# jinli99/iShapEditing

Hardware: AMD Instinct MI355X
Metric: end-to-end drag-edit wall-clock (s) per shape (lower is better)
Workload: dtype f16

## Files before the change

### ishapediting_amd/csrc/igemm.hip

```cpp
#include "common.h"
#include "igemm_epilogue.h"
#include "gn_bwd_terms.h"

template <int BM, int BN, int BK, int WM, int WN, bool CONV3>
__global__ __launch_bounds__(256) void igemm_kernel(IgemmArgs a) {
  constexpr int CPR = BK / 8;
  constexpr int XL = BM * CPR / 256;
  constexpr int WL = BN * CPR / 256;
  constexpr int TMW = BM / WM, TNW = BN / WN;
  constexpr int MT = TMW / 16, NT = TNW / 16;
  static_assert(XL >= 1 && WL >= 1, "tile too small for 256 threads");
  extern __shared__ __attribute__((aligned(16))) char smem_raw[];
  half_t* sX = reinterpret_cast<half_t*>(smem_raw);
  half_t* sW = sX + 2 * BM * BK;

  const int tid = threadIdx.x;
  const int lane = tid & 63;
  const int wave = tid >> 6;
  const int wm = wave / WN, wn = wave % WN;
  const int m0 = blockIdx.x * BM;
  const int n0 = blockIdx.y * BN;
  const int batch = blockIdx.z / a.ksplit;
  const int ks_id = blockIdx.z % a.ksplit;

// ... 220 lines not shown
  hipEvent_t e;
  (void)hipEventCreate(&e);
  return e;
}
extern "C" int ishap_profile_begin(void) {
  for (auto& r : g_prof) { g_prof_pool.push_back(r.a); g_prof_pool.push_back(r.b); if (r.c) g_prof_pool.push_back(r.c); }
  g_prof.clear();
  g_prof_on = true;
  return 0;
}
extern "C" int ishap_profile_end(double* out, int nvar) {
  g_prof_on = false;
  for (int i = 0; i < nvar * 3; ++i) out[i] = 0.0;
  for (auto& r : g_prof) {
    if (hipEventSynchronize(r.b) != hipSuccess) return -1;
    float ms = 0.f;
    if (hipEventElapsedTime(&ms, r.a, r.b) != hipSuccess) return -1;
    if (r.variant < nvar) { out[r.variant * 3] += 1.0; out[r.variant * 3 + 1] += ms; out[r.variant * 3 + 2] += r.flops; }
  }
  return 0;
}

#include <map>
#include <cstring>
#include <array>
#include <string>
extern "C" int ishap_profile_shapes(char* buf, int cap) {
  std::map<std::array<int, 6>, std::array<double, 4>> agg;
  for (auto& r : g_prof) {
    if (hipEventSynchronize(r.c ? r.c : r.b) != hipSuccess) return -1;
    float ms = 0.f, ms2 = 0.f;
    if (hipEventElapsedTime(&ms, r.a, r.b) != hipSuccess) return -1;
    if (r.c && hipEventElapsedTime(&ms2, r.b, r.c) != hipSuccess) return -1;
    auto& v = agg[{r.M, r.N, r.K, r.conv3, r.big ? 128 : 64, r.ksplit}];
    v[0] += 1.0; v[1] += ms; v[2] += ms2; v[3] += r.flops * 1e-9;
  }
  std::string out;
  char line[160];
  for (auto& kv : agg) {
    snprintf(line, sizeof line, "%d,%d,%d,%d,%d,%d,%.0f,%.4f,%.4f,%.3f\n", kv.first[0], kv.first[1], kv.first[2], kv.first[3],
             kv.first[4], kv.first[5], kv.second[0], kv.second[1], kv.second[2], kv.second[3]);
    out += line;
  }
  if ((int)out.size() + 1 > cap) return -2;
  memcpy(buf, out.c_str(), out.size() + 1);
  return (int)agg.size();
}

int igemm2_launch_main(const IgemmArgs& a, bool big, hipStream_t s);
bool igemm2_two_teams(const IgemmArgs& a, bool big);
bool igemm4_applicable(const IgemmArgs& a, bool big);
bool igemm4_two_teams(const IgemmArgs& a, bool big);
bool igemm4_tall_tiles(const IgemmArgs& a, bool big);
int igemm4_launch_main(const IgemmArgs& a, bool big, hipStream_t s);
static bool igemm4_wanted(const IgemmArgs& a, bool big) {
  static const int use4 = [] { const char* e = getenv("ISHAP_IGEMM4"); return e ? atoi(e) : 2; }();
  return use4 && (use4 > 1 || big) && igemm4_applicable(a, big);
}

template <int BM, int BN, int BK, int WM, int WN, bool CONV3>
static int launch_cfg(const IgemmArgs& a, hipStream_t s) {
  int prof_slot = -1;
  auto fire = [&]() -> int {
    if constexpr (BK == 64) {
      if (CONV3 && igemm4_wanted(a, BM == 128)) return igemm4_launch_main(a, BM == 128, s);
      return igemm2_launch_main(a, BM == 128, s);
    } else {
      constexpr size_t smem = 2 * (size_t)(BM + BN) * BK * sizeof(half_t);
      auto kern = igemm_kernel<BM, BN, BK, WM, WN, CONV3>;
      ISHAP_TRY(ishap_set_max_lds((const void*)kern, (int)smem));
      const dim3 grid(a.M / BM, ceil_div(a.N, BN), a.nbatch * a.ksplit);
      if (g_igemm_prof_start) hipExtLaunchKernelGGL(kern, grid, dim3(256), smem, s, g_igemm_prof_start, g_igemm_prof_stop, 0, a);
      else hipLaunchKernelGGL(kern, grid, dim3(256), smem, s, a);
      return 0;
    }
  };
  if (g_prof_on) {
    ProfRec r;
    r.a = prof_event(); r.b = prof_event(); r.c = nullptr;
    r.flops = 2.0 * a.M * a.N * a.K * a.nbatch * a.flops_scale;
    r.variant = BK == 64 ? ((CONV3 ? 0 : 2) + (BM == 128 ? 0 : 1)) : 6;
    if (BK == 64 && igemm2_two_teams(a, BM == 128)) r.variant = 4;
    if (BK == 64 && CONV3 && igemm4_wanted(a, BM == 128))
      r.variant = BM == 128 ? 8 : (a.W == 8 ? 11 : (igemm4_tall_tiles(a, false) ? 12 : (igemm4_two_teams(a, false) ? 10 : 9)));
    r.M = a.M * a.nbatch; r.N = a.N; r.K = a.K; r.conv3 = CONV3; r.big = BM == 128; r.ksplit = a.ksplit;
    g_igemm_prof_start = r.a; g_igemm_prof_stop = r.b;
    const int rc = fire();
    g_igemm_prof_start = nullptr; g_igemm_prof_stop = nullptr;
    if (rc) return rc;
    prof_slot = (int)g_prof.size();
    g_prof.push_back(r);
  } else {
    ISHAP_TRY(fire());
  }
  ISHAP_CHECK_HIP(hipGetLastError());
  if (a.ksplit > 1 && !a.defer_reduce) {
    const unsigned rblocks = (unsigned)((long long)a.nbatch * (a.M / 16) * ((a.N + 63) / 64));
    hipLaunchKernelGGL(igemm_splitk_reduce, dim3(rblocks), dim3(256), 0, s, a);
    ISHAP_CHECK_HIP(hipGetLastError());
    if (prof_slot >= 0) {
      g_prof[prof_slot].c = prof_event();
      (void)hipEventRecord(g_prof[prof_slot].c, s);
    }
  }
  return 0;
}

static bool igemm_use_big(int M, int N, int nbatch) {
  if (M % 128 != 0 || N < 128) return false;
  long long blocks = (long long)(M / 128) * ceil_div(N, 128) * nbatch;
  static const int big_min = [] { const char* e = getenv("ISHAP_BIG_MIN"); return e ? atoi(e) : 192; }();
  return blocks >= big_min;
}
int igemm_pick_ksplit(int M, int N, int K, int nbatch, bool pending) {
  const bool big = igemm_use_big(M, N, nbatch);
  const int bm = big ? 128 : 64, bn = big ? 128 : 64;
  long long blocks = (long long)(M / bm) * ceil_div(N, bn) * nbatch;
  int ks = K / 64;
  constexpr int nosplit = 36;
  constexpr int fill = 224;
  constexpr int minsteps = 6;
  constexpr int p_nosplit = 12, p_minsteps = 3;
  if (ks < (pending ? p_nosplit : nosplit)) return 1;
  int split = 1;
  while (blocks * split < fill && ks / (split * 2) >= (pending ? p_minsteps : minsteps) && split < 32) split *= 2;
  return split;
}

int igemm_reduce_launch(const IgemmArgs& a, hipStream_t s) {
  ISHAP_REQUIRE(a.ksplit > 1 && a.ws && a.M % 16 == 0 && a.N % 4 == 0, "reduce: split-K slices of a finished launch");
  const unsigned rblocks = (unsigned)((long long)a.nbatch * (a.M / 16) * ((a.N + 63) / 64));
  hipLaunchKernelGGL(igemm_splitk_reduce, dim3(rblocks), dim3(256), 0, s, a);
  ISHAP_CHECK_HIP(hipGetLastError());
  return 0;
}

bool igemm_skinny_applicable(const IgemmArgs& a);
// ... 57 lines not shown
```

### ishapediting_amd/csrc/igemm4.hip

```cpp
#include "common.h"
#include "igemm_epilogue.h"
#include <type_traits>

__device__ __attribute__((aligned(128))) half_t g_zero_line4[64];
typedef __attribute__((address_space(3))) void lds_void4;

constexpr int ig4_loads(int a, int b, int wi, int xi) {
  int c = 0;
  for (int u = a; u <= b; ++u) c += wi + ((u % 3 == 0) ? xi : 0);
  return c;
}

#ifndef IG4_PRO
#define IG4_PRO 2
#endif

#ifdef ABL_NOLOAD
#define IG4_DMA(src, dst) asm volatile("" ::"v"(src), "v"((unsigned)(unsigned long long)(lds_void4*)(dst)))
#else
#define IG4_DMA(src, dst) __builtin_amdgcn_global_load_lds((src), (lds_void4*)(dst), 16, 0, 0)
#endif

__device__ __forceinline__ void ig4_wait_vm(int n) {
#define IG4_W(k) case k: asm volatile("s_waitcnt vmcnt(" #k ")" ::: "memory"); break;
  switch (n) {
    IG4_W(0) IG4_W(1) IG4_W(2) IG4_W(3) IG4_W(4) IG4_W(5) IG4_W(6) IG4_W(7) IG4_W(8) IG4_W(9) IG4_W(10) IG4_W(11) IG4_W(12)
    IG4_W(13) IG4_W(14) IG4_W(15) IG4_W(16) IG4_W(17) IG4_W(18) IG4_W(19) IG4_W(20) IG4_W(21) IG4_W(22) IG4_W(23) IG4_W(24)
    IG4_W(25) IG4_W(26) IG4_W(27) IG4_W(28) IG4_W(29) IG4_W(30) IG4_W(31) IG4_W(32) IG4_W(33) IG4_W(34) IG4_W(35) IG4_W(36)
    IG4_W(37) IG4_W(38) IG4_W(39) IG4_W(40)
    default: asm volatile("s_waitcnt vmcnt(0)" ::: "memory"); break;
  }
#undef IG4_W
}

template <int BM, int BN, int WD, int NSTW, int NSTX, int HALVES = 1>
__global__ __launch_bounds__(512 * HALVES) void igemm4_kernel(const void* hX, const void* hWt, int hK, int hCin, int hldx, int hldw, int hH, int hW,
                                                              int hksplit, int hnwg, unsigned hpacked, int hbase, IgemmArgs a) {
  const IgemmHot h{(const half_t*)hX, (const half_t*)hWt, hK, hCin, hldx, hldw, hH, hW, hksplit, hnwg, hpacked};
#if defined(__HIP_DEVICE_COMPILE__)
  constexpr int BK = 64;
  constexpr int XI = BM / 8 / 4;
  constexpr int WI = BN / 8 / 4;
  constexpr int WSLOT = BN * BK;
  constexpr int XSLOT = (BM + 8) * BK;
  constexpr int RING = NSTW * WSLOT + NSTX * XSLOT;
  constexpr int TMW = BM / 2, TNW = BN / 2, MT = TMW / 16, NT = TNW / 16;
  constexpr int DIST = NSTW - 1;
  constexpr int PRO = DIST < IG4_PRO ? DIST : IG4_PRO;
  constexpr int RAMP = DIST - PRO;
  static_assert(RAMP <= 6, "ramp iterations are peeled by hand");
  static_assert(NSTX * 3 >= DIST + 3, "activation ring too shallow for the prefetch distance");
  static_assert(BM % WD == 0, "a tile is whole image rows (fragment addresses are per lane, so a 16-pixel MFMA sub-tile may span rows)");
  static_assert(DIST * (WI + XI) <= 40, "ig4_wait_vm covers up to 40 outstanding loads");
  extern __shared__ __attribute__((aligned(16))) char smem_raw[];

  const int tid = threadIdx.x, lane = tid & 63;
  const int wave_all = __builtin_amdgcn_readfirstlane(tid >> 6);
  const int team = HALVES == 2 ? wave_all >> 3 : 0;
  const int wave8 = wave_all & 7;
  half_t* const sW = reinterpret_cast<half_t*>(smem_raw) + team * RING;
  half_t* const sX = sW + NSTW * WSLOT;
  const bool loader = wave8 >= 4;
  const int wave = wave8 & 3;
  const int wm = wave >> 1, wn = wave & 1;
  IG_STAMP(0, wave_all == 0);
  if (tid < HALVES * NSTX * 8) {
    const int tm = tid / (NSTX * 8), k = tid - tm * (NSTX * 8);
    *reinterpret_cast<f32x4*>(reinterpret_cast<half_t*>(smem_raw) + tm * RING + NSTW * WSLOT + (k >> 3) * XSLOT + BM * BK + (k & 7) * 8) =
        (f32x4){0.f, 0.f, 0.f, 0.f};
  }
  int tile_m, tile_n, tile_z;
  {
    const int nx = h.ny_shift() >= 0 ? (1 << h.nx_shift()) : (int)gridDim.x, ny = h.ny_shift() >= 0 ? (1 << h.ny_shift()) : (int)gridDim.y;
    const int nwg = h.nwg;
    const bool n_outer = (hbase >> 30) & 1;
    const int lin = (hbase & 0x3fffffff) + blockIdx.x + nx * (blockIdx.y + ny * blockIdx.z);
    const int q = nwg >> 3, r = nwg & 7, xcd = lin & 7, pos = lin >> 3;
    const int swz = (xcd < r ? xcd * (q + 1) : r * (q + 1) + (xcd - r) * q) + pos;
    if (n_outer) {
      tile_m = swz & (nx - 1);
      const int rest = swz >> h.nx_shift();
      tile_n = rest / h.ksplit;
      tile_z = rest - tile_n * h.ksplit;
    } else if (h.ny_shift() >= 0) {
      tile_n = swz & (ny - 1);
      tile_m = (swz >> h.ny_shift()) & (nx - 1);
      tile_z = swz >> (h.ny_shift() + h.nx_shift());
    } else {
      tile_n = swz % ny;
      tile_m = (swz / ny) % nx;
      tile_z = swz / (ny * nx);
    }
  }
  const int m0 = tile_m * BM, n0 = tile_n * BN;
  const int ks_id = tile_z;
  const int H = h.H, HW = H * WD;
  const int NC = h.Cin / BK;
  const int NC2 = (int)(h.packed >> 25);
  const int G = 3 * NC;
  const int per = (G + h.ksplit - 1) / h.ksplit, per2 = (NC2 + h.ksplit - 1) / h.ksplit;
  int g0 = min(G, ks_id * per), g1 = min(G, g0 + per);
  int c20 = min(NC2, ks_id * per2), c21 = min(NC2, c20 + per2);
  int nk_loop = (g1 - g0) * 3 + (c21 - c20);
  if (HALVES == 2) {
    const int ga = min(g1 - g0, (nk_loop + 3) / 6);
    const int n0s = ga * 3, n1s = nk_loop - n0s;
    nk_loop = max(n0s, n1s);
    if (team == 0) { g1 = g0 + ga; c21 = c20; }
    else g0 += ga;
  }
  const int ns3 = (g1 - g0) * 3, ns = ns3 + (c21 - c20);
  const int n_img = h.hw_shift() >= 0 ? (m0 >> h.hw_shift()) : m0 / HW;
  const int y0 = (m0 - n_img * HW) / WD;
  __syncthreads();

  f32x4 acc[NT][MT];
#pragma unroll
  for (int i = 0; i < NT; ++i)
#pragma unroll
    for (int j = 0; j < MT; ++j) acc[i][j] = (f32x4){0.f, 0.f, 0.f, 0.f};

  IG_STAMP(1, wave_all == 0);
  if (loader) {
    const int lrow = lane >> 3, pch = lane & 7;
    int hc = g0 / 3, hdy = g0 - hc * 3, hdx = 0;
    const half_t* xp[XI];
    const half_t* zp[XI];
    int yr[XI], xc[XI];
#pragma unroll
    for (int i = 0; i < XI; ++i) {
      const int row = (wave * XI + i) * 8 + lrow;
      yr[i] = y0 + row / WD;
      xc[i] = row % WD;
      const int sc = (pch ^ (row & 7)) * 8;
      zp[i] = (const half_t*)g_zero_line4 + sc;
      xp[i] = h.X + ((long long)n_img * HW + (long long)(yr[i] + hdy - 1) * WD + xc[i]) * h.ldx + hc * BK + sc;
    }
    const long long x_row = (long long)WD * h.ldx;
    const half_t* wp[WI];
#pragma unroll
    for (int i = 0; i < WI; ++i) {
      const int row = (wave * WI + i) * 8 + lrow;
      wp[i] = h.Wt + (long long)(n0 + row) * h.ldw + (pch ^ ((row >> 1) & 7)) * 8 + (long long)(3 * hdy) * h.Cin + hc * BK;
    }
    int hws = 0, hxs = 0;
    int issued = 0, tot = 0;
// ... 258 lines not shown
          if (decltype(SLAB_ENDS)::value && s + 1 >= ns3) read_half(integral_constant<int, 1>{}, 0, sw_off, sx_off, xa, wa);
          else read_half(integral_constant<int, (d + 1) % 3>{}, 0, sw_off, sx_off, xa, wa);
        }
        __builtin_amdgcn_sched_barrier(0);
      }
      mfma_half(xb, wb);
    };
    auto step = [&](auto DX, auto SLAB_ENDS, int s) __attribute__((always_inline)) {
      if constexpr (INTERLEAVE) step_il(DX, SLAB_ENDS, s);
      else step_burst(DX, SLAB_ENDS, s);
    };
    if (nk_loop > 0) __builtin_amdgcn_s_barrier();
    asm volatile("" ::: "memory");
    IG_STAMP(2, wave_all == 0);
    if (ns > 0) {
      if (ns3 > 0) read_half(integral_constant<int, 0>{}, 0, sw_off, sx_off, xa, wa);
      else read_half(integral_constant<int, 1>{}, 0, sw_off, sx_off, xa, wa);
    }
    int s = 0;
    for (; s < ns3; s += 3) {
      step(integral_constant<int, 0>{}, std::false_type{}, s);
      step(integral_constant<int, 1>{}, std::false_type{}, s + 1);
      step(integral_constant<int, 2>{}, std::true_type{}, s + 2);
    }
    for (; s < ns; ++s) step(integral_constant<int, 1>{}, std::true_type{}, s);
    for (; s < nk_loop; ++s)
      if (s + 1 < nk_loop) __builtin_amdgcn_s_barrier();
  }
  IG_STAMP(3, wave_all == 0);
  const bool merge_in_epilogue = HALVES == 2 && igemm_epilogue_is_staged(a, 0);
  if (HALVES == 2 && !merge_in_epilogue) {
    f32x4* red = reinterpret_cast<f32x4*>(reinterpret_cast<half_t*>(smem_raw) + RING);
    __syncthreads();
    if (!loader && team == 1) {
#pragma unroll
      for (int i = 0; i < NT; ++i)
#pragma unroll
        for (int j = 0; j < MT; ++j) red[((i * MT + j) * 4 + wave) * 64 + lane] = acc[i][j];
    }
    __syncthreads();
    if (!loader && team == 0) {
#pragma unroll
      for (int i = 0; i < NT; ++i)
#pragma unroll
        for (int j = 0; j < MT; ++j) acc[i][j] += red[((i * MT + j) * 4 + wave) * 64 + lane];
    }
  }
  IG_STAMP(4, wave_all == 0);
  igemm_epilogue<MT, NT, TMW, TNW, BN, 512 * HALVES>(a, acc, m0, n0, wm, wn, lane, 0, ks_id, reinterpret_cast<float*>(smem_raw),
                                                     !loader && (team == 0 || merge_in_epilogue), merge_in_epilogue ? team : -1);
#endif
}

template <int BM, int BN, int WD, int NSTW, int NSTX, int HALVES = 1>
static int launch4(const IgemmArgs& a, hipStream_t s) {
  constexpr size_t ring = (size_t)HALVES * (NSTW * BN * 64 + NSTX * (BM + 8) * 64) * sizeof(half_t);
  constexpr size_t epi = (size_t)HALVES * BM * (BN + 4) * 4 + (size_t)BM * (BN + 8) * 2 + 16384;
  static_assert((ring > epi ? ring : epi) <= 163840, "LDS");
  const size_t smem = ring > epi ? ring : epi;
  auto kern = igemm4_kernel<BM, BN, WD, NSTW, NSTX, HALVES>;
  ISHAP_TRY(ishap_set_max_lds((const void*)kern, (int)smem));
  const dim3 grid(a.M / BM, ceil_div(a.N, BN), a.ksplit);
  IgemmArgs b = a;
  auto lg2 = [](int v) { int k = 0; while ((1 << k) < v) ++k; return (1 << k) == v ? k : -1; };
  b.w_shift = lg2(a.W);
  b.hw_shift = lg2(a.H * a.W);
  if (b.w_shift < 0 || b.hw_shift < 0) b.w_shift = b.hw_shift = -1;
  b.nx_shift = lg2((int)grid.x);
  b.ny_shift = lg2((int)grid.y);
  if (b.nx_shift < 0 || b.ny_shift < 0) b.nx_shift = b.ny_shift = -1;
  IgemmHot h;
  h.X = b.X; h.Wt = b.Wt; h.K = b.K; h.Cin = b.Cin; h.ldx = b.ldx; h.ldw = b.ldw; h.H = b.H; h.W = b.W; h.ksplit = b.ksplit;
  h.nwg = (int)(grid.x * grid.y * grid.z);
  h.packed = (unsigned)(b.w_shift & 0x3f) | (unsigned)(b.hw_shift & 0x3f) << 6 | (unsigned)(b.nx_shift & 0x3f) << 12 |
             (unsigned)(b.ny_shift & 0x3f) << 18 | (b.ups ? 1u << 24 : 0u) | (unsigned)(b.K2 / 64) << 25;
  int n_outer = 0;
  if (b.nx_shift >= 0) {
    static const int force = [] { const char* e = getenv("ISHAP_IG4_NOUTER"); return e ? atoi(e) : 2; }();
    const int nx = (int)grid.x, ny = (int)grid.y, nz = (int)grid.z;
    const int q = (h.nwg + 7) / 8;
    const double wp = (double)BN * (b.K / (double)nz) * 2.0;
    const double xs = (double)BM * b.Cin * 2.0 / nz + (b.K2 ? (double)BM * b.K2 * 2.0 / nz : 0.0);
    auto cdiv = [](int a, int d) { return (a + d - 1) / d; };
    const int nA = ny < q ? ny : q, mzA = cdiv(q, ny), mA = nx < mzA ? nx : mzA, zA = cdiv(mzA, nx);
    const double costA = (double)nA * zA * wp + (double)mA * zA * xs;
    const int mB = nx < q ? nx : q, znB = cdiv(q, nx), zB = nz < znB ? nz : znB;
    const double costB = (double)znB * wp + (double)mB * zB * xs;
    n_outer = force == 2 ? (costB < 0.8 * costA) : force;
  }
  const int order_bit = n_outer ? (1 << 30) : 0;
  const int tiles = h.nwg;
  const int chunk = a.chunk_tiles;
  const bool chunked = chunk > 0 && chunk % 8 == 0 && tiles > chunk && b.nx_shift >= 0 && !g_igemm_prof_start;
  if (chunked) {
    for (int base = 0; base < tiles; base += chunk) {
      const int n = tiles - base < chunk ? tiles - base : chunk;
      hipLaunchKernelGGL(kern, dim3(n), dim3(512 * HALVES), smem, s,
                         (const void*)h.X, (const void*)h.Wt, h.K, h.Cin, h.ldx, h.ldw, h.H, h.W, h.ksplit, h.nwg, h.packed, base | order_bit, b);
    }
  } else if (g_igemm_prof_start) hipExtLaunchKernelGGL(kern, grid, dim3(512 * HALVES), smem, s, g_igemm_prof_start, g_igemm_prof_stop, 0,
                                                (const void*)h.X, (const void*)h.Wt, h.K, h.Cin, h.ldx, h.ldw, h.H, h.W, h.ksplit, h.nwg, h.packed, order_bit, b);
  else hipLaunchKernelGGL(kern, grid, dim3(512 * HALVES), smem, s,
                          (const void*)h.X, (const void*)h.Wt, h.K, h.Cin, h.ldx, h.ldw, h.H, h.W, h.ksplit, h.nwg, h.packed, order_bit, b);
  ISHAP_CHECK_HIP(hipGetLastError());
  return 0;
}

bool igemm4_applicable(const IgemmArgs& a, bool big) {
  const int BM = big ? 128 : 64;
  if (!a.conv3 || a.nbatch != 1 || a.Cin % 64 != 0 || a.K != 9 * a.Cin + a.K2) return false;
  if (a.K2 && (a.K2 % 64 != 0 || a.K2 / 64 > 127 || !a.X2)) return false;
  const bool w8 = !big && a.W == 8 && a.H == 8 && a.ksplit > 1;
  if (a.K2 && !big && !w8) return false;
  if (big ? (a.W != 128 && a.W != 64 && a.W != 32 && a.W != 16) : (a.W != 16 && a.W != 32 && a.W != 64 && !w8)) return false;
  if (BM % a.W != 0 || (a.H * a.W) % BM != 0 || a.M % BM != 0) return false;
  return true;
}

int igemm4_small_map_slices(const IgemmArgs& a) {
  static const int on = [] { const char* all = getenv("ISHAP_IGEMM4"); return (all ? atoi(all) : 2) > 1; }();
  constexpr int target = 256;
  if (!on || !a.conv3 || a.W != 8 || a.H != 8 || a.nbatch != 1 || a.Cin % 64 != 0 || a.M % 64 != 0 || a.K != 9 * a.Cin + a.K2) return 0;
  if (a.K2 && (a.K2 % 64 != 0 || a.K2 / 64 > 127 || !a.X2)) return 0;
  const int tiles = (a.M / 64) * ((a.N + 63) / 64), G = 3 * (a.Cin / 64);
  int ks = (target + tiles / 2) / tiles;
  if (ks > 16) ks = 16;
  if (ks > G) ks = G;
  if (ks < 2) return 0;
  const int per = (G + ks - 1) / ks;
  return (G + per - 1) / per;
}

#ifndef IG4_BIG_W
#define IG4_BIG_W 5
#define IG4_BIG_X 3
#endif
#ifndef IG4_SMALL_W
#define IG4_SMALL_W 6
#define IG4_SMALL_X 3
#endif
#ifndef IG4_W8_W
#define IG4_W8_W 4
#define IG4_W8_X 3
#endif
#ifndef IG4_TEAM_W
#define IG4_TEAM_W 6
#define IG4_TEAM_X 3
#endif
bool igemm4_two_teams(const IgemmArgs& a, bool big) {
  static const int on = [] { const char* e = getenv("ISHAP_IG4_TEAMS"); return e ? atoi(e) : 2; }();
  if (big || on != 2) return false;
  const long long tiles = (long long)(a.M / 64) * ((a.N + 63) / 64) * a.ksplit;
  const int groups = (3 * (a.Cin / 64) + a.ksplit - 1) / a.ksplit;
  return tiles <= 256 && 3 * groups + a.K2 / 64 >= 48;
}
bool igemm4_tall_tiles(const IgemmArgs& a, bool big) {
  static const int on = [] { const char* e = getenv("ISHAP_IG4_TEAMS"); return e ? atoi(e) : 2; }();
  if (big || !on || a.W != 64 || a.K2 != 0 || a.ksplit != 1 || a.M % 128 != 0 || (a.H * a.W) % 128 != 0) return false;
  const long long tiles = (long long)(a.M / 128) * ((a.N + 63) / 64);
  return tiles >= 224 && tiles <= 512;
}
int igemm4_launch_main(const IgemmArgs& a, bool big, hipStream_t s) {
  if (big) {
    if (a.W == 128) return launch4<128, 128, 128, IG4_BIG_W, IG4_BIG_X>(a, s);
    if (a.W == 64) return launch4<128, 128, 64, IG4_BIG_W, IG4_BIG_X>(a, s);
    if (a.W == 32) return launch4<128, 128, 32, IG4_BIG_W, IG4_BIG_X>(a, s);
    return launch4<128, 128, 16, IG4_BIG_W, IG4_BIG_X>(a, s);
  }
  if (igemm4_tall_tiles(a, big)) return launch4<128, 64, 64, IG4_SMALL_W, IG4_SMALL_X>(a, s);
#ifdef IG4_TALL_PROBE
  if ((a.W == 32 || a.W == 16) && a.K2 == 0 && a.M % 128 == 0 && (a.H * a.W) % 128 == 0) {
    const int st = 3 * ((3 * (a.Cin / 64) + a.ksplit - 1) / a.ksplit);
    if (st >= 9 && st <= 12) return a.W == 32 ? launch4<128, 64, 32, IG4_W8_W, IG4_W8_X>(a, s) : launch4<128, 64, 16, IG4_W8_W, IG4_W8_X>(a, s);
    return a.W == 32 ? launch4<128, 64, 32, IG4_SMALL_W, IG4_SMALL_X>(a, s) : launch4<128, 64, 16, IG4_SMALL_W, IG4_SMALL_X>(a, s);
  }
#endif
  if (igemm4_two_teams(a, big)) {
    if (a.W == 64) return launch4<64, 64, 64, IG4_TEAM_W, IG4_TEAM_X, 2>(a, s);
    if (a.W == 32) return launch4<64, 64, 32, IG4_TEAM_W, IG4_TEAM_X, 2>(a, s);
    if (a.W == 8) return launch4<64, 64, 8, IG4_W8_W, IG4_W8_X>(a, s);
    return launch4<64, 64, 16, IG4_TEAM_W, IG4_TEAM_X, 2>(a, s);
  }
  if (a.W == 8) return launch4<64, 64, 8, IG4_W8_W, IG4_W8_X>(a, s);
  const int steps = 3 * ((3 * (a.Cin / 64) + a.ksplit - 1) / a.ksplit);
  if (a.K2 == 0 && steps >= 9 && steps <= 12) {
    if (a.W == 64) return launch4<64, 64, 64, IG4_W8_W, IG4_W8_X>(a, s);
    if (a.W == 32) return launch4<64, 64, 32, IG4_W8_W, IG4_W8_X>(a, s);
    return launch4<64, 64, 16, IG4_W8_W, IG4_W8_X>(a, s);
  }
  if (a.W == 64) return launch4<64, 64, 64, IG4_SMALL_W, IG4_SMALL_X>(a, s);
  if (a.W == 32) return launch4<64, 64, 32, IG4_SMALL_W, IG4_SMALL_X>(a, s);
  return launch4<64, 64, 16, IG4_SMALL_W, IG4_SMALL_X>(a, s);
}
```

### ishapediting_amd/csrc/igemm_epilogue.h

```cpp
#pragma once
#include "common.h"
#include "gn_bwd_terms.h"
#include "gn_act.h"
#include <type_traits>

#ifdef IG_STAMPS
extern __device__ unsigned long long* g_ig_stamps;
#define IG_STAMP(slot, cond)                                                                                   \
  do {                                                                                                         \
    if (cond) {                                                                                                \
      unsigned long long t_;                                                                                   \
      __builtin_amdgcn_sched_barrier(0);                                                                       \
      asm volatile("s_memtime %0\n\ts_waitcnt lgkmcnt(0)" : "=s"(t_)::"memory");                              \
      __builtin_amdgcn_sched_barrier(0);                                                                       \
      if ((threadIdx.x & 63) == 0)                                                                             \
        g_ig_stamps[(size_t)(blockIdx.x + gridDim.x * (blockIdx.y + gridDim.y * blockIdx.z)) * 16 + (slot)] = t_; \
    }                                                                                                          \
  } while (0)
#else
#define IG_STAMP(slot, cond) do {} while (0)
#endif

__device__ __forceinline__ bool igemm_epilogue_is_staged(const IgemmArgs& a, int batch) {
  const half_t* out16 = (const half_t*)a.out + (long long)batch * a.bso;
  const bool aligned16 = ((reinterpret_cast<unsigned long long>(out16) | reinterpret_cast<unsigned long long>(a.res)) & 15) == 0;
  return a.out_mode == IG_OUT_F16 && a.ksplit == 1 && (a.N & 7) == 0 && (a.ldo & 7) == 0 && (!a.res || (a.ldr & 7) == 0) && aligned16 &&
         (!a.gb_x || (a.N & 31) == 0);
}

template <int MT, int NT, int TMW, int TNW, int BN, int T>
__device__ __forceinline__ void igemm_epilogue_staged(const IgemmArgs& a, f32x4 (&acc)[NT][MT], int m0, int n0, int wm, int wn,
                                                      int lane, int batch, float* lds_f, bool active, int team2) {
  constexpr int BM_T = 2 * TMW;
  constexpr int LDF = BN + 4;
  constexpr int LDH = BN + 8;
  constexpr int CPRW = BN / 8;
  constexpr int ITEMS = BM_T * CPRW;
  constexpr int RPT = (ITEMS + T - 1) / T;
  constexpr int RSTEP = T / CPRW;
  constexpr int NW = T / 64;
  constexpr int PAIRS = BN / 2;
  constexpr int PARTS = (T / PAIRS) < (BM_T / 8) ? (T / PAIRS) : (BM_T / 8);
  constexpr int RPP = BM_T / PARTS;
  static_assert(T % CPRW == 0 && (ITEMS % T == 0 || ITEMS < T) && BM_T % PARTS == 0, "thread <-> tile mappings");
  const bool two = team2 >= 0;
  float* const tileF = lds_f;
  half_t* const tileH = reinterpret_cast<half_t*>(lds_f + (two ? 2 : 1) * BM_T * LDF);
  float* const slots = reinterpret_cast<float*>(tileH + BM_T * LDH);
  const int t = threadIdx.x;
  const bool stamp_wave = active && wm == 0 && wn == 0;
  (void)stamp_wave;
  IG_STAMP(5, stamp_wave);
  __syncthreads();
  if (active) {
    float* const mine = tileF + (two ? team2 * BM_T * LDF : 0);
#pragma unroll
    for (int j = 0; j < MT; ++j)
#pragma unroll
      for (int i = 0; i < NT; ++i)
        *reinterpret_cast<f32x4*>(mine + (wm * TMW + j * 16 + (lane & 15)) * LDF + wn * TNW + i * 16 + (lane >> 4) * 4) = acc[i][j];
  }
  const int chunk = t % CPRW, row_first = t / CPRW;
  const int n = n0 + chunk * 8;
  const bool has = row_first < BM_T && n < a.N;
  const float alpha = a.alpha;
  const int HW = a.H * a.W;
  half_t* const out16 = (half_t*)a.out + (long long)batch * a.bso;
  f32x4 b1[2] = {{0.f, 0.f, 0.f, 0.f}, {0.f, 0.f, 0.f, 0.f}}, b2[2] = {{0.f, 0.f, 0.f, 0.f}, {0.f, 0.f, 0.f, 0.f}};
  half8 rr[RPT];
  const bool want_fwd = a.stat_out != nullptr, want_gb = a.gb_x != nullptr;
  if (has) {
    if (a.bias) { b1[0] = *reinterpret_cast<const f32x4*>(a.bias + n); b1[1] = *reinterpret_cast<const f32x4*>(a.bias + n + 4); }
    if (a.bias2) { b2[0] = *reinterpret_cast<const f32x4*>(a.bias2 + n); b2[1] = *reinterpret_cast<const f32x4*>(a.bias2 + n + 4); }
    if (a.res) {
#pragma unroll
      for (int k = 0; k < RPT; ++k) {
        const int m = m0 + row_first + k * RSTEP;
        long long rrow = m;
        if (a.res_ups) {
          int img, py, px;
          if (a.hw_shift >= 0) { img = m >> a.hw_shift; const int p = m & (HW - 1); py = p >> a.w_shift; px = p & (a.W - 1); }
          else { img = m / HW; const int p = m - img * HW; py = p / a.W; px = p - py * a.W; }
          rrow = (long long)img * (HW >> 2) + (py >> 1) * (a.W >> 1) + (px >> 1);
        }
        rr[k] = *reinterpret_cast<const half8*>(a.res + rrow * a.ldr + n);
      }
// ... 82 lines not shown
      *reinterpret_cast<f32x4*>(slots + (part * PAIRS + pair) * 4) = (f32x4){s0, q0, s1, q1};
    }
    IG_STAMP(8, stamp_wave);
    __syncthreads();
    IG_STAMP(9, stamp_wave);
    if (t < BN * 2) {
      const int nl = t >> 1, k = t & 1;
      if (n0 + nl < a.N) {
        double S = 0.0, Q = 0.0;
#pragma unroll
        for (int part = 0; part < PARTS; ++part) {
          const f32x4 r = *reinterpret_cast<const f32x4*>(slots + (part * PAIRS + (nl >> 1)) * 4);
          S += (double)r[(nl & 1) * 2];
          Q += (double)r[(nl & 1) * 2 + 1];
        }
        const double P = (double)(float)tileH[nl], nn = (double)BM_T;
        const double v = k ? Q + P * (2.0 * S + nn * P) : S + nn * P;
#ifdef ABL_STAT_COPIES
        atomicAdd(reinterpret_cast<unsigned long long*>(a.stat_out + (long long)((m0 / BM_T) % ABL_STAT_COPIES) * a.N * 2 +
                                                        ((long long)n_img * a.N + n0 + nl) * 2 + k),
#else
        atomicAdd(reinterpret_cast<unsigned long long*>(a.stat_out + ((long long)n_img * a.N + n0 + nl) * 2 + k),
#endif
                  (unsigned long long)__double2ll_rn(v * (double)(k ? STAT_SCALE_SQ : STAT_SCALE_SUM)));
      }
    }
  } else {
#pragma unroll
    for (int c = 0; c < 8; ++c) {
#pragma unroll
      for (int o = CPRW; o < 64; o <<= 1) { gs1[c] += __shfl_xor(gs1[c], o); gs2[c] += __shfl_xor(gs2[c], o); }
    }
    IG_STAMP(8, stamp_wave);
    if (lane < CPRW) {
      float* dst = slots + ((t >> 6) * BN + lane * 8) * 2;
#pragma unroll
      for (int c = 0; c < 8; ++c) { dst[c * 2] = gs1[c]; dst[c * 2 + 1] = gs2[c]; }
    }
    __syncthreads();
    if (t < BN * 2) {
      const int nl = t >> 1, k = t & 1;
      if (n0 + nl < a.N) {
        double v = 0.0;
#pragma unroll
        for (int w = 0; w < NW; ++w) v += (double)slots[(w * BN + nl) * 2 + k];
        atomicAdd(reinterpret_cast<unsigned long long*>(a.gb_csums + ((long long)n_img * a.N + n0 + nl) * 2 + k),
                  (unsigned long long)__double2ll_rn(v * (double)STAT_SCALE_SUM));
      }
    }
  }
  IG_STAMP(10, stamp_wave);
}

template <int MT, int NT, int TMW, int TNW, int BN, int STAGE_THREADS = 0>
__device__ __forceinline__ void igemm_epilogue(const IgemmArgs& a, f32x4 (&acc)[NT][MT], int m0, int n0, int wm, int wn,
                                               int lane, int batch, int ks_id, float* lds_f, bool active = true, int team2 = -1) {
  const float alpha = a.alpha;
  const int out_mode = a.out_mode;
  const float* const bias = a.bias;
  const float* const bias2 = a.bias2;
  const half_t* const resp = a.res;
  const int HW = a.H * a.W;
  constexpr int BM_T = 2 * TMW;
  constexpr int LDT = BN + 8;
  half_t* const out16 = (half_t*)a.out + (long long)batch * a.bso;
  if constexpr (STAGE_THREADS > 0) {
    if (igemm_epilogue_is_staged(a, batch)) {
      igemm_epilogue_staged<MT, NT, TMW, TNW, BN, STAGE_THREADS>(a, acc, m0, n0, wm, wn, lane, batch, lds_f, active, team2);
      return;
    }
  }
  constexpr bool staged = false;
  half_t* const tile = reinterpret_cast<half_t*>(lds_f);
  const bool stamp_wave = active && wm == 0 && wn == 0;
  (void)stamp_wave;
  IG_STAMP(5, stamp_wave);
  if (staged) __syncthreads();
  IG_STAMP(6, stamp_wave);
  float ssum[NT][4], ssq[NT][4], piv[NT][4];
#pragma unroll
  for (int i = 0; i < NT; ++i)
#pragma unroll
    for (int c = 0; c < 4; ++c) { ssum[i][c] = 0.f; ssq[i][c] = 0.f; piv[i][c] = 0.f; }
  auto col = [&](int i) { return n0 + wn * TNW + i * 16 + (lane >> 4) * 4; };
  auto row = [&](int j) { return m0 + wm * TMW + j * 16 + (lane & 15); };
  if (!active) {
  } else if (a.ksplit > 1) {
#pragma unroll
    for (int j = 0; j < MT; ++j) {
      float* dst = a.ws + (((long long)ks_id * a.nbatch + batch) * a.M + row(j)) * a.N;
#pragma unroll
      for (int i = 0; i < NT; ++i)
        if (col(i) < a.N) *reinterpret_cast<f32x4*>(dst + col(i)) = acc[i][j];
    }
  } else {
    f32x4 b1[NT], b2[NT];
    half4 rr[2][NT];
    int pimg[MT], ppy[MT], ppx[MT];
#pragma unroll
    for (int i = 0; i < NT; ++i) {
      b1[i] = (f32x4){0.f, 0.f, 0.f, 0.f};
      b2[i] = (f32x4){0.f, 0.f, 0.f, 0.f};
      if (col(i) < a.N) {
        if (bias) b1[i] = *reinterpret_cast<const f32x4*>(bias + col(i));
        if (bias2) b2[i] = *reinterpret_cast<const f32x4*>(bias2 + col(i));
      }
    }
#pragma unroll
    for (int j = 0; j < MT; ++j) {
      const int m = row(j);
      pimg[j] = 0; ppy[j] = 0; ppx[j] = 0;
      if (a.res_ups || out_mode == IG_OUT_NCHW_F32) {
        pimg[j] = m / HW;
        const int p = m - pimg[j] * HW;
        ppy[j] = p / a.W;
        ppx[j] = p - ppy[j] * a.W;
      }
    }
    auto fetch_res = [&](int j) {
      if (!resp || j >= MT) return;
      const long long rrow = a.res_ups ? ((long long)pimg[j] * (HW >> 2) + (ppy[j] >> 1) * (a.W >> 1) + (ppx[j] >> 1)) : row(j);
// ... 104 lines not shown
#pragma unroll
      for (int j = 0; j < MT; ++j) {
        const int m = m0 + wm * TMW + j * 16 + (lane & 15);
        const half4 xv = *reinterpret_cast<const half4*>(a.gb_x + (long long)m * a.N + n);
#pragma unroll
        for (int c = 0; c < 4; ++c) {
          float dyh, xhat;
          gn_bwd_term(acc[i][j][c], (float)xv[c], mu[c], rs[c], gam[c], bet[c], esc[c], esh[c], a.gb_film != 0, a.gb_act != 0, dyh, xhat);
          ssum[i][c] += dyh;
          ssq[i][c] += dyh * xhat;
        }
      }
    }
  }
  if ((a.stat_out || a.gb_x) && a.ksplit == 1) {
    long long* const sdst = a.gb_x ? a.gb_csums : a.stat_out;
    const float scale_q = a.gb_x ? STAT_SCALE_SUM : STAT_SCALE_SQ;
    const bool pivoted = !a.gb_x;
#pragma unroll
    for (int i = 0; i < NT; ++i)
#pragma unroll
      for (int c = 0; c < 4; ++c) {
        if (pivoted) {
          const float P = row16_max(piv[i][c]);
          const float e = piv[i][c] - P;
          ssq[i][c] = fmaf(e, fmaf((float)MT, e, 2.f * ssum[i][c]), ssq[i][c]);
          ssum[i][c] = fmaf((float)MT, e, ssum[i][c]);
          piv[i][c] = P;
        }
        ssum[i][c] = row16_sum(ssum[i][c]);
        ssq[i][c] = row16_sum(ssq[i][c]);
      }
    IG_STAMP(9, stamp_wave);
    __syncthreads();
    if (active && (lane & 15) == 0) {
#pragma unroll
      for (int i = 0; i < NT; ++i)
#pragma unroll
        for (int c = 0; c < 4; ++c) {
          const int nl = wn * TNW + i * 16 + (lane >> 4) * 4 + c;
          lds_f[(wm * BN + nl) * 3 + 0] = ssum[i][c];
          lds_f[(wm * BN + nl) * 3 + 1] = ssq[i][c];
          lds_f[(wm * BN + nl) * 3 + 2] = piv[i][c];
        }
    }
    __syncthreads();
    const int t = threadIdx.x;
    if (t < BN * 2) {
      const int nl = t >> 1;
      if (n0 + nl < a.N) {
        constexpr double nW = 16.0 * MT;
        double v = 0.0;
#pragma unroll
        for (int w = 0; w < 2; ++w) {
          const double sw = (double)lds_f[(w * BN + nl) * 3 + 0], qw = (double)lds_f[(w * BN + nl) * 3 + 1];
          const double P = (double)lds_f[(w * BN + nl) * 3 + 2];
          v += (t & 1) ? qw + P * (2.0 * sw + nW * P) : sw + nW * P;
        }
        const int n_img = m0 / HW;
        const long long fx = __double2ll_rn(v * (double)((t & 1) ? scale_q : STAT_SCALE_SUM));
#ifdef ABL_STAT_COPIES
        atomicAdd(reinterpret_cast<unsigned long long*>(sdst + (long long)((m0 / BM_T) % ABL_STAT_COPIES) * a.N * 2 +
                                                        ((long long)n_img * a.N + n0 + nl) * 2 + (t & 1)),
#else
        atomicAdd(reinterpret_cast<unsigned long long*>(sdst + ((long long)n_img * a.N + n0 + nl) * 2 + (t & 1)),
#endif
                  (unsigned long long)fx);
      }
    }
  }
  IG_STAMP(10, stamp_wave);
}
```

Baseline: 0.1629.

## Add halo-tile implicit-GEMM conv3 kernel reusing input rows across the nine taps

Adds a new igemm4 halo kernel for 3x3 convolutions. Each 128-pixel tile of whole image rows loads one input slab with a one-row halo per channel chunk, and all nine filter taps read shifted offsets from that slab. Before, the X tile was re-fetched for every tap. The kernel has compile-time vmcnt schedules and a 4-wave M split with BN=32, and the epilogue gains a WM template parameter to match. It is enabled by default for mid-size grids (224-256 tiles), at the cost of added complexity and an extra LDS footprint for the halo rows.

```diff
diff --git a/ishapediting_amd/csrc/igemm.hip b/ishapediting_amd/csrc/igemm.hip
--- a/ishapediting_amd/csrc/igemm.hip
+++ b/ishapediting_amd/csrc/igemm.hip
@@ -296,6 +296,7 @@
 bool igemm4_applicable(const IgemmArgs& a, bool big);
 bool igemm4_two_teams(const IgemmArgs& a, bool big);
 bool igemm4_tall_tiles(const IgemmArgs& a, bool big);
+bool igemm4_halo_tiles(const IgemmArgs& a, bool big);
 int igemm4_launch_main(const IgemmArgs& a, bool big, hipStream_t s);
 static bool igemm4_wanted(const IgemmArgs& a, bool big) {
   static const int use4 = [] { const char* e = getenv("ISHAP_IGEMM4"); return e ? atoi(e) : 2; }();
@@ -326,7 +327,7 @@
     r.variant = BK == 64 ? ((CONV3 ? 0 : 2) + (BM == 128 ? 0 : 1)) : 6;
     if (BK == 64 && igemm2_two_teams(a, BM == 128)) r.variant = 4;
     if (BK == 64 && CONV3 && igemm4_wanted(a, BM == 128))
-      r.variant = BM == 128 ? 8 : (a.W == 8 ? 11 : (igemm4_tall_tiles(a, false) ? 12 : (igemm4_two_teams(a, false) ? 10 : 9)));
+      r.variant = BM == 128 ? 8 : (a.W == 8 ? 11 : igemm4_halo_tiles(a, false) ? 7 : (igemm4_tall_tiles(a, false) ? 12 : (igemm4_two_teams(a, false) ? 10 : 9)));
     r.M = a.M * a.nbatch; r.N = a.N; r.K = a.K; r.conv3 = CONV3; r.big = BM == 128; r.ksplit = a.ksplit;
     g_igemm_prof_start = r.a; g_igemm_prof_stop = r.b;
     const int rc = fire();
diff --git a/ishapediting_amd/csrc/igemm4.hip b/ishapediting_amd/csrc/igemm4.hip
--- a/ishapediting_amd/csrc/igemm4.hip
+++ b/ishapediting_amd/csrc/igemm4.hip
@@ -1,6 +1,7 @@
 #include "common.h"
 #include "igemm_epilogue.h"
 #include <type_traits>
+#include <utility>
 
 __device__ __attribute__((aligned(128))) half_t g_zero_line4[64];
 typedef __attribute__((address_space(3))) void lds_void4;
@@ -31,6 +32,29 @@
     default: asm volatile("s_waitcnt vmcnt(0)" ::: "memory"); break;
   }
 #undef IG4_W
+}
+
+__device__ __forceinline__ void ig4_tile(const IgemmHot& h, int hbase, int& tile_m, int& tile_n, int& tile_z) {
+  const int nx = h.ny_shift() >= 0 ? (1 << h.nx_shift()) : (int)gridDim.x, ny = h.ny_shift() >= 0 ? (1 << h.ny_shift()) : (int)gridDim.y;
+  const int nwg = h.nwg;
+  const bool n_outer = (hbase >> 30) & 1;
+  const int lin = (hbase & 0x3fffffff) + blockIdx.x + nx * (blockIdx.y + ny * blockIdx.z);
+  const int q = nwg >> 3, r = nwg & 7, xcd = lin & 7, pos = lin >> 3;
+  const int swz = (xcd < r ? xcd * (q + 1) : r * (q + 1) + (xcd - r) * q) + pos;
+  if (n_outer) {
+    tile_m = swz & (nx - 1);
+    const int rest = swz >> h.nx_shift();
+    tile_n = rest / h.ksplit;
+    tile_z = rest - tile_n * h.ksplit;
+  } else if (h.ny_shift() >= 0) {
+    tile_n = swz & (ny - 1);
+    tile_m = (swz >> h.ny_shift()) & (nx - 1);
+    tile_z = swz >> (h.ny_shift() + h.nx_shift());
+  } else {
+    tile_n = swz % ny;
+    tile_m = (swz / ny) % nx;
+    tile_z = swz / (ny * nx);
+  }
 }
 
 template <int BM, int BN, int WD, int NSTW, int NSTX, int HALVES = 1>
@@ -70,28 +94,7 @@
         (f32x4){0.f, 0.f, 0.f, 0.f};
   }
   int tile_m, tile_n, tile_z;
-  {
-    const int nx = h.ny_shift() >= 0 ? (1 << h.nx_shift()) : (int)gridDim.x, ny = h.ny_shift() >= 0 ? (1 << h.ny_shift()) : (int)gridDim.y;
-    const int nwg = h.nwg;
-    const bool n_outer = (hbase >> 30) & 1;
-    const int lin = (hbase & 0x3fffffff) + blockIdx.x + nx * (blockIdx.y + ny * blockIdx.z);
-    const int q = nwg >> 3, r = nwg & 7, xcd = lin & 7, pos = lin >> 3;
-    const int swz = (xcd < r ? xcd * (q + 1) : r * (q + 1) + (xcd - r) * q) + pos;
-    if (n_outer) {
-      tile_m = swz & (nx - 1);
-      const int rest = swz >> h.nx_shift();
-      tile_n = rest / h.ksplit;
-      tile_z = rest - tile_n * h.ksplit;
-    } else if (h.ny_shift() >= 0) {
-      tile_n = swz & (ny - 1);
-      tile_m = (swz >> h.ny_shift()) & (nx - 1);
-      tile_z = swz >> (h.ny_shift() + h.nx_shift());
-    } else {
-      tile_n = swz % ny;
-      tile_m = (swz / ny) % nx;
-      tile_z = swz / (ny * nx);
-    }
-  }
+  ig4_tile(h, hbase, tile_m, tile_n, tile_z);
   const int m0 = tile_m * BM, n0 = tile_n * BN;
   const int ks_id = tile_z;
   const int H = h.H, HW = H * WD;
@@ -456,13 +459,239 @@
 #endif
 }
 
-template <int BM, int BN, int WD, int NSTW, int NSTX, int HALVES = 1>
+constexpr int ig4h_min(int a, int b) { return a < b ? a : b; }
+constexpr int ig4h_wupto(int S, int NS, int DIST, int PRO) { return ig4h_min(NS, ig4h_min(S + 1 + DIST, PRO + 2 * (S + 1))); }
+constexpr int ig4h_xpart(int S, int NCH, int XI) {
+  const int p = S % 9, XP = (XI + 1) / 2;
+  return (S / 9 + 1 < NCH && p < XP) ? ig4h_min(2, XI - 2 * p) : 0;
+}
+constexpr int ig4h_issued(int S, int NCH, int XI, int WI, int DIST, int PRO) {
+  int n = XI + WI * ig4h_wupto(S, 9 * NCH, DIST, PRO);
+  for (int t = 0; t <= S; ++t) n += ig4h_xpart(t, NCH, XI);
+  return n;
+}
+constexpr int ig4h_wait(int S, int NCH, int XI, int WI, int DIST, int PRO) {
+  const int NS = 9 * NCH;
+  int J = -1;
+  while (ig4h_wupto(J, NS, DIST, PRO) <= S) ++J;
+  int posx = 0;
+  for (int t = 0; t < J; ++t) posx += ig4h_xpart(t, NCH, XI);
+  int need = XI + WI * (S + 1) + posx;
+  if (S % 9 == 0 && S > 0) {
+    const int last = S - 9 + (XI + 1) / 2 - 1;
+    const int px = ig4h_issued(last, NCH, XI, WI, DIST, PRO);
+    need = need > px ? need : px;
+  }
+  return ig4h_issued(S - 1, NCH, XI, WI, DIST, PRO) - need;
+}
+constexpr bool ig4h_classes(int XI, int WI, int DIST, int PRO) {
+  for (int p = 0; p < 9; ++p) {
+    const int first = ig4h_wait(p, 2, XI, WI, DIST, PRO), mid = ig4h_wait(9 + p, 3, XI, WI, DIST, PRO), last = ig4h_wait(9 + p, 2, XI, WI, DIST, PRO);
+    if (first != ig4h_wait(p, 6, XI, WI, DIST, PRO) || last != ig4h_wait(45 + p, 6, XI, WI, DIST, PRO) || last != ig4h_wait(18 + p, 3, XI, WI, DIST, PRO)) return false;
+    for (int k = 1; k < 5; ++k)
+      if (mid != ig4h_wait(9 * k + p, 6, XI, WI, DIST, PRO)) return false;
+  }
+  return true;
+}
+template <class F, int... P>
+__device__ __forceinline__ void ig4h_unroll(F&& f, std::integer_sequence<int, P...>) {
+  (f(std::integral_constant<int, P>{}), ...);
+}
+
+template <int WD, int NSTW>
+__global__ __launch_bounds__(512) void igemm4_halo_kernel(const void* hX, const void* hWt, int hK, int hCin, int hldx, int hldw, int hH, int hW,
+                                                          int hksplit, int hnwg, unsigned hpacked, int hbase, IgemmArgs a) {
+  const IgemmHot h{(const half_t*)hX, (const half_t*)hWt, hK, hCin, hldx, hldw, hH, hW, hksplit, hnwg, hpacked};
+#if defined(__HIP_DEVICE_COMPILE__)
+  constexpr int BM = 128, BN = 32, BK = 64;
+  constexpr int R = BM / WD;
+  constexpr int SR = (R + 2) * WD;
+  constexpr int XI = SR / 8 / 4;
+  constexpr int XP = (XI + 1) / 2;
+  constexpr int WI = 1;
+  constexpr int WSLOT = BN * BK;
+  constexpr int XSLOT = (SR + 8) * BK;
+  constexpr int TMW = 32, TNW = 32, MT = 2, NT = 2;
+  constexpr int DIST = NSTW - 1;
+  constexpr int PRO = DIST < IG4_PRO ? DIST : IG4_PRO;
+  static_assert(WD % 8 == 0 && BM % WD == 0 && SR % 32 == 0, "a tile is whole image rows; the swizzle survives a shift by WD");
+  static_assert(ig4h_classes(XI, WI, DIST, PRO), "a slice's first / middle / last chunks wait as the model slices the loader uses");
+  extern __shared__ __attribute__((aligned(16))) char smem_raw[];
+
+  const int tid = threadIdx.x, lane = tid & 63;
+  const int wave8 = __builtin_amdgcn_readfirstlane(tid >> 6);
+  half_t* const sW = reinterpret_cast<half_t*>(smem_raw);
+  half_t* const sX = sW + NSTW * WSLOT;
+  const bool loader = wave8 >= 4;
+  const int wave = wave8 & 3;
+  IG_STAMP(0, wave8 == 0);
+  if (tid < 2 * 8)
+    *reinterpret_cast<f32x4*>(sX + (tid >> 3) * XSLOT + SR * BK + (tid & 7) * 8) = (f32x4){0.f, 0.f, 0.f, 0.f};
+  int tile_m, tile_n, tile_z;
+  ig4_tile(h, hbase, tile_m, tile_n, tile_z);
+  const int m0 = tile_m * BM, n0 = tile_n * BN;
+  const int ks_id = tile_z;
+  const int H = h.H, HW = H * WD;
+  const int NC = h.Cin / BK;
+  const int per = (NC + h.ksplit - 1) / h.ksplit;
+  const int c0 = min(NC, ks_id * per), nch = min(NC, c0 + per) - c0;
+  const int ns = 9 * nch;
+  const int n_img = h.hw_shift() >= 0 ? (m0 >> h.hw_shift()) : m0 / HW;
+  const int y0 = (m0 - n_img * HW) / WD;
+  __syncthreads();
+
+  f32x4 acc[NT][MT];
+#pragma unroll
+  for (int i = 0; i < NT; ++i)
+#pragma unroll
+    for (int j = 0; j < MT; ++j) acc[i][j] = (f32x4){0.f, 0.f, 0.f, 0.f};
+
+  IG_STAMP(1, wave8 == 0);
+  if (loader) {
+    using std::integral_constant;
+    const int lrow = lane >> 3, pch = lane & 7;
+    const half_t* xp[XI];
+    int xinc[XI];
+#pragma unroll
+    for (int i = 0; i < XI; ++i) {
+      const int sr = (wave * XI + i) * 8 + lrow;
+      const int yy = y0 - 1 + sr / WD, xx = sr % WD;
+      const int sc = (pch ^ (sr & 7)) * 8;
+      const bool ok = (unsigned)yy < (unsigned)H;
+      const long long pix = h.ups() ? (long long)n_img * (HW >> 2) + (yy >> 1) * (WD >> 1) + (xx >> 1) : (long long)n_img * HW + yy * WD + xx;
+      xp[i] = ok ? h.X + pix * h.ldx + c0 * BK + sc : (const half_t*)g_zero_line4 + sc;
+      xinc[i] = ok ? BK : 0;
+    }
+    const int wrow = wave * 8 + lrow;
+    const half_t* wp = h.Wt + (long long)(n0 + wrow) * h.ldw + (pch ^ ((wrow >> 1) & 7)) * 8 + c0 * BK;
+    int hws = 0;
+    unsigned hx = 0;
+    auto issue_w = [&](auto U) __attribute__((always_inline)) {
+      IG4_DMA(wp, sW + hws * WSLOT + wave * 8 * BK);
+      hws = hws + 1 == NSTW ? 0 : hws + 1;
+      wp += decltype(U)::value % 9 == 8 ? (long long)BK - 8LL * h.Cin : (long long)h.Cin;
+    };
+    auto issue_x = [&](auto I) __attribute__((always_inline)) {
+      constexpr int i = decltype(I)::value;
+      IG4_DMA(xp[i], sX + hx * XSLOT + (wave * XI + i) * 8 * BK);
+      xp[i] += xinc[i];
+      if constexpr (i == XI - 1) hx ^= 1u;
+    };
+    if (nch > 0) {
+      ig4h_unroll(issue_x, std::make_integer_sequence<int, XI>{});
+      ig4h_unroll(issue_w, std::make_integer_sequence<int, PRO>{});
+    }
+    auto iter = [&](auto SC, auto NCHC) __attribute__((always_inline)) {
+      constexpr int S = decltype(SC)::value, NCH = decltype(NCHC)::value;
+      constexpr int cnt = ig4h_wait(S, NCH, XI, WI, DIST, PRO);
+      static_assert(cnt >= 0 && cnt <= 63, "vmcnt range");
+      asm volatile("s_waitcnt vmcnt(%0)" ::"n"(cnt) : "memory");
+      __builtin_amdgcn_s_barrier();
+      asm volatile("" ::: "memory");
+      constexpr int w0 = ig4h_wupto(S - 1, 9 * NCH, DIST, PRO), w1 = ig4h_wupto(S, 9 * NCH, DIST, PRO);
+      ig4h_unroll([&](auto U) __attribute__((always_inline)) { issue_w(integral_constant<int, w0 + decltype(U)::value>{}); },
+                  std::make_integer_sequence<int, w1 - w0>{});
+      constexpr int xn = ig4h_xpart(S, NCH, XI), xi0 = 2 * (S % 9);
+      ig4h_unroll([&](auto I) __attribute__((always_inline)) { issue_x(integral_constant<int, xi0 + decltype(I)::value>{}); },
+                  std::make_integer_sequence<int, xn>{});
+    };
+    auto chunk = [&](auto BASE, auto NCHC) __attribute__((always_inline)) {
+      ig4h_unroll([&](auto P) __attribute__((always_inline)) { iter(integral_constant<int, decltype(BASE)::value + decltype(P)::value>{}, NCHC); },
+                  std::make_integer_sequence<int, 9>{});
+    };
+    if (nch == 1) {
+      chunk(integral_constant<int, 0>{}, integral_constant<int, 1>{});
+    } else if (nch > 1) {
+      chunk(integral_constant<int, 0>{}, integral_constant<int, 2>{});
+      for (int k = 1; k + 1 < nch; ++k) chunk(integral_constant<int, 9>{}, integral_constant<int, 3>{});
+      chunk(integral_constant<int, 9>{}, integral_constant<int, 2>{});
+    }
+  } else {
+    unsigned wo[2][NT], xo[3][3][2][MT];
+    const unsigned wbase = (unsigned)(unsigned long long)(lds_void4*)sW, xbase = (unsigned)(unsigned long long)(lds_void4*)sX;
+#pragma unroll
+    for (int kk = 0; kk < 2; ++kk) {
+      const int ch = (lane >> 4) + 4 * kk;
+#pragma unroll
+      for (int i = 0; i < NT; ++i) {
+        const int row = i * 16 + (lane & 15);
+        wo[kk][i] = wbase + 2 * (row * BK + ((ch ^ ((row >> 1) & 7)) * 8));
+      }
+#pragma unroll
+      for (int j = 0; j < MT; ++j) {
+        const int pl = wave * TMW + j * 16 + (lane & 15);
+        const int x = pl % WD;
+#pragma unroll
+        for (int dy = 0; dy < 3; ++dy)
+#pragma unroll
+          for (int dx = 0; dx < 3; ++dx) {
+            const int xs = x + dx - 1;
+            const int row = (xs >= 0 && xs < WD) ? pl + dy * WD + dx - 1 : SR;
+            xo[dy][dx][kk][j] = xbase + 2 * (row * BK + (row == SR ? ch * 8 : ((ch ^ (row & 7)) * 8)));
+          }
+      }
+    }
+    half8 xa[MT], wa[NT], xb[MT], wb[NT];
+    unsigned sw_off = 0, sx_off = 0;
+    auto read_half = [&](const unsigned (&xs)[2][MT], int kk, half8 (&xf)[MT], half8 (&wf)[NT]) __attribute__((always_inline)) {
+#pragma unroll
+      for (int j = 0; j < MT; ++j) asm volatile("ds_read_b128 %0, %1" : "=v"(xf[j]) : "v"(xs[kk][j] + sx_off) : "memory");
+#pragma unroll
+      for (int i = 0; i < NT; ++i) asm volatile("ds_read_b128 %0, %1" : "=v"(wf[i]) : "v"(wo[kk][i] + sw_off) : "memory");
+    };
+    auto wait_frags = [&](auto pending, half8 (&xf)[MT], half8 (&wf)[NT]) __attribute__((always_inline)) {
+      asm volatile("s_waitcnt lgkmcnt(%4)" : "+v"(xf[0]), "+v"(xf[1]), "+v"(wf[0]), "+v"(wf[1]) : "n"(decltype(pending)::value) : "memory");
+    };
+    auto mfma_half = [&](half8 (&xf)[MT], half8 (&wf)[NT]) __attribute__((always_inline)) {
+#pragma unroll
+      for (int i = 0; i < NT; ++i)
+#pragma unroll
+        for (int j = 0; j < MT; ++j) acc[i][j] = __builtin_amdgcn_mfma_f32_16x16x32_f16(wf[i], xf[j], acc[i][j], 0, 0, 0);
+    };
+    using std::integral_constant;
+    auto step = [&](auto TC, int s) __attribute__((always_inline)) {
+      constexpr int T = decltype(TC)::value, TN = (T + 1) % 9;
+      read_half(xo[T / 3][T % 3], 1, xb, wb);
+      wait_frags(integral_constant<int, MT + NT>{}, xa, wa);
+      __builtin_amdgcn_sched_barrier(0);
+      mfma_half(xa, wa);
+      __builtin_amdgcn_sched_barrier(0);
+      wait_frags(integral_constant<int, 0>{}, xb, wb);
+      sw_off = sw_off + WSLOT * 2 == NSTW * WSLOT * 2 ? 0u : sw_off + WSLOT * 2;
+      if constexpr (T == 8) sx_off ^= XSLOT * 2;
+      if (s + 1 < ns) {
+        __builtin_amdgcn_s_barrier();
+        asm volatile("" ::: "memory");
+        read_half(xo[TN / 3][TN % 3], 0, xa, wa);
+        __builtin_amdgcn_sched_barrier(0);
+      }
+      mfma_half(xb, wb);
+    };
+    if (ns > 0) __builtin_amdgcn_s_barrier();
+    asm volatile("" ::: "memory");
+    IG_STAMP(2, wave8 == 0);
+    if (ns > 0) read_half(xo[0][0], 0, xa, wa);
+    for (int s = 0; s < ns; s += 9)
+      ig4h_unroll([&](auto TC) __attribute__((always_inline)) { step(TC, s + decltype(TC)::value); }, std::make_integer_sequence<int, 9>{});
+  }
+  IG_STAMP(3, wave8 == 0);
+  IG_STAMP(4, wave8 == 0);
+  igemm_epilogue<MT, NT, TMW, TNW, BN, 512, 4>(a, acc, m0, n0, wave, 0, lane, 0, ks_id, reinterpret_cast<float*>(smem_raw), !loader, -1);
+#endif
+}
+
+template <int BM, int BN, int WD, int NSTW, int NSTX, int HALVES = 1, bool HALO = false>
 static int launch4(const IgemmArgs& a, hipStream_t s) {
-  constexpr size_t ring = (size_t)HALVES * (NSTW * BN * 64 + NSTX * (BM + 8) * 64) * sizeof(half_t);
+  static_assert(!HALO || (BM == 128 && BN == 32 && NSTX == 2 && HALVES == 1), "the halo kernel's tile");
+  constexpr int XROWS = HALO ? (BM / WD + 2) * WD : BM;
+  constexpr size_t ring = (size_t)HALVES * (NSTW * BN * 64 + NSTX * (XROWS + 8) * 64) * sizeof(half_t);
   constexpr size_t epi = (size_t)HALVES * BM * (BN + 4) * 4 + (size_t)BM * (BN + 8) * 2 + 16384;
   static_assert((ring > epi ? ring : epi) <= 163840, "LDS");
   const size_t smem = ring > epi ? ring : epi;
-  auto kern = igemm4_kernel<BM, BN, WD, NSTW, NSTX, HALVES>;
+  auto kern = [] {
+    if constexpr (HALO) return igemm4_halo_kernel<WD, NSTW>;
+    else return igemm4_kernel<BM, BN, WD, NSTW, NSTX, HALVES>;
+  }();
   ISHAP_TRY(ishap_set_max_lds((const void*)kern, (int)smem));
   const dim3 grid(a.M / BM, ceil_div(a.N, BN), a.ksplit);
   IgemmArgs b = a;
@@ -564,6 +793,17 @@
   const long long tiles = (long long)(a.M / 128) * ((a.N + 63) / 64);
   return tiles >= 224 && tiles <= 512;
 }
+#ifndef IG4_HALO_W
+#define IG4_HALO_W 6
+#endif
+bool igemm4_halo_tiles(const IgemmArgs& a, bool big) {
+  static const int on = [] { const char* e = getenv("ISHAP_IG4_HALO"); return e ? atoi(e) : 1; }();
+  if (big || !on || a.K2 != 0 || (a.W != 64 && a.W != 32 && a.W != 16) || a.M % 128 != 0 || (a.H * a.W) % 128 != 0 || a.N % 32 != 0) return false;
+  const int nc = a.Cin / 64;
+  if (nc % a.ksplit != 0 || nc / a.ksplit < 2) return false;
+  const long long tiles = (long long)(a.M / 128) * (a.N / 32) * a.ksplit;
+  return tiles >= 224 && tiles <= 256;
+}
 int igemm4_launch_main(const IgemmArgs& a, bool big, hipStream_t s) {
   if (big) {
     if (a.W == 128) return launch4<128, 128, 128, IG4_BIG_W, IG4_BIG_X>(a, s);
@@ -571,6 +811,11 @@
     if (a.W == 32) return launch4<128, 128, 32, IG4_BIG_W, IG4_BIG_X>(a, s);
     return launch4<128, 128, 16, IG4_BIG_W, IG4_BIG_X>(a, s);
   }
+  if (igemm4_halo_tiles(a, big)) {
+    if (a.W == 64) return launch4<128, 32, 64, IG4_HALO_W, 2, 1, true>(a, s);
+    if (a.W == 32) return launch4<128, 32, 32, IG4_HALO_W, 2, 1, true>(a, s);
+    return launch4<128, 32, 16, IG4_HALO_W, 2, 1, true>(a, s);
+  }
   if (igemm4_tall_tiles(a, big)) return launch4<128, 64, 64, IG4_SMALL_W, IG4_SMALL_X>(a, s);
 #ifdef IG4_TALL_PROBE
   if ((a.W == 32 || a.W == 16) && a.K2 == 0 && a.M % 128 == 0 && (a.H * a.W) % 128 == 0) {
diff --git a/ishapediting_amd/csrc/igemm_epilogue.h b/ishapediting_amd/csrc/igemm_epilogue.h
--- a/ishapediting_amd/csrc/igemm_epilogue.h
+++ b/ishapediting_amd/csrc/igemm_epilogue.h
@@ -28,10 +28,10 @@
          (!a.gb_x || (a.N & 31) == 0);
 }
 
-template <int MT, int NT, int TMW, int TNW, int BN, int T>
+template <int MT, int NT, int TMW, int TNW, int BN, int T, int WM = 2>
 __device__ __forceinline__ void igemm_epilogue_staged(const IgemmArgs& a, f32x4 (&acc)[NT][MT], int m0, int n0, int wm, int wn,
                                                       int lane, int batch, float* lds_f, bool active, int team2) {
-  constexpr int BM_T = 2 * TMW;
+  constexpr int BM_T = WM * TMW;
   constexpr int LDF = BN + 4;
   constexpr int LDH = BN + 8;
   constexpr int CPRW = BN / 8;
@@ -220,7 +220,7 @@
   IG_STAMP(10, stamp_wave);
 }
 
-template <int MT, int NT, int TMW, int TNW, int BN, int STAGE_THREADS = 0>
+template <int MT, int NT, int TMW, int TNW, int BN, int STAGE_THREADS = 0, int WM = 2>
 __device__ __forceinline__ void igemm_epilogue(const IgemmArgs& a, f32x4 (&acc)[NT][MT], int m0, int n0, int wm, int wn,
                                                int lane, int batch, int ks_id, float* lds_f, bool active = true, int team2 = -1) {
   const float alpha = a.alpha;
@@ -229,12 +229,12 @@
   const float* const bias2 = a.bias2;
   const half_t* const resp = a.res;
   const int HW = a.H * a.W;
-  constexpr int BM_T = 2 * TMW;
+  constexpr int BM_T = WM * TMW;
   constexpr int LDT = BN + 8;
   half_t* const out16 = (half_t*)a.out + (long long)batch * a.bso;
   if constexpr (STAGE_THREADS > 0) {
     if (igemm_epilogue_is_staged(a, batch)) {
-      igemm_epilogue_staged<MT, NT, TMW, TNW, BN, STAGE_THREADS>(a, acc, m0, n0, wm, wn, lane, batch, lds_f, active, team2);
+      igemm_epilogue_staged<MT, NT, TMW, TNW, BN, STAGE_THREADS, WM>(a, acc, m0, n0, wm, wn, lane, batch, lds_f, active, team2);
       return;
     }
   }
@@ -445,7 +445,7 @@
         constexpr double nW = 16.0 * MT;
         double v = 0.0;
 #pragma unroll
-        for (int w = 0; w < 2; ++w) {
+        for (int w = 0; w < WM; ++w) {
           const double sw = (double)lds_f[(w * BN + nl) * 3 + 0], qw = (double)lds_f[(w * BN + nl) * 3 + 1];
           const double P = (double)lds_f[(w * BN + nl) * 3 + 2];
           v += (t & 1) ? qw + P * (2.0 * sw + nW * P) : sw + nW * P;
```

New measurement: 0.1593 (median of 6 runs). 1.02x faster.
